# modal-labs/modal-examples

Hardware: AMD Instinct MI355X
Metric: SDXL 1024px images/sec (whole node) (higher is better)
Workload: dtype bf16; 1 GPU; model=sdxl-base-unet-2.6b, global_batch=16, image=1024x1024, denoise_steps=4, parallelism=dp1, hipgraph=True

## Files before the change

### modal_examples_amd/ops/csrc/attention_fwd32.hip

```cpp
#include "attention_mfma32.h"

#include <cstdlib>

#define FA32_NWAVES 4

template <int D, bool CAUSAL, int KVB, bool DEFER>
__global__ __launch_bounds__(FA32_NWAVES * WAVE)
__attribute__((amdgpu_waves_per_eu((D == 64 && CAUSAL) ? 3 : 1)))
void fa32_kernel(
    const short* __restrict__ Q, const short* __restrict__ K,
    const short* __restrict__ V, short* __restrict__ O,
    float* __restrict__ LSE, int B, int Hq, int Hkv, int Sq, int Sk,
    float scale, AttnFwdStrides st) {
  constexpr int KROW = D + FA_PPAD;
  constexpr int DCH = D / 16;
  constexpr int DT = D / 32;
  constexpr int QBLK = 32 * FA32_NWAVES;
  constexpr int KF = KVB / 32;

  __shared__ alignas(16) short Ks[KVB][KROW];
  __shared__ alignas(16) short Vs[KVB][KROW];

  const int tid = threadIdx.x;
  const int w = tid / WAVE;
  const int l = tid % WAVE;
  const int l31 = l & 31;
  const int hi5 = l >> 5;

  const int qblk = blockIdx.x;
  const int h = blockIdx.y;
  const int b = blockIdx.z;
  const int hkv = h / (Hq / Hkv);

  const long long qoff = b * st.q.b + h * st.q.h;
  const long long koff = b * st.k.b + hkv * st.k.h;
  const long long voff = b * st.v.b + hkv * st.v.h;
  const long long ooff = b * st.o.b + h * st.o.h;
  const int q0 = qblk * QBLK + w * 32;
  const int my_q = q0 + l31;
  const int causal_off = Sk - Sq;

  bf16x8 qreg[DCH];
  const long long qrow_off = qoff + (long long)my_q * st.q.s;
  const bool q_ok = my_q < Sq;
#pragma unroll
  for (int c = 0; c < DCH; ++c) {
    qreg[c] = q_ok
        ? *(const bf16x8*)&Q[qrow_off + c * 16 + hi5 * 8]
        : bf16x8_zero();
  }

  f32x16 acc[DT];
#pragma unroll
  for (int dt = 0; dt < DT; ++dt)
#pragma unroll
    for (int r = 0; r < 16; ++r) acc[dt][r] = 0.f;
  float m_run = -1e30f, l_run = 0.f;

  int nkb = (Sk + KVB - 1) / KVB;
  if (CAUSAL) {
    int max_kv = qblk * QBLK + QBLK - 1 + causal_off;
    int lim = (max_kv + KVB) / KVB;
    if (lim < nkb) nkb = lim;
  }

  constexpr int NT = FA32_NWAVES * WAVE;
  bf16x8 kreg[KVB * (D / 8) / NT], vreg[KVB * (D / 8) / NT];
  auto load_chunks = [&](int kb) {
    stage_load<D, KVB, NT>(K + koff, st.k.s, V + voff, st.v.s, kb * KVB, Sk,
                           tid, kreg, vreg);
  };
  auto write_chunks = [&]() {
    stage_write<D, KVB, NT>(&Ks[0][0], &Vs[0][0], tid, kreg, vreg);
  };

  load_chunks(0);
  for (int kb = 0; kb < nkb; ++kb) {
    __syncthreads();
    write_chunks();
    __syncthreads();
    if (kb + 1 < nkb) load_chunks(kb + 1);

    f32x16 s[KF];
#pragma unroll
    for (int f = 0; f < KF; ++f)
#pragma unroll
      for (int r = 0; r < 16; ++r) s[f][r] = 0.f;
#pragma unroll
    for (int f = 0; f < KF; ++f) {
#pragma unroll
      for (int c = 0; c < DCH; ++c) {
        bf16x8 kfrag = row_frag<KROW>(&Ks[0][0], f * 32 + l31, hi5, c);
        __builtin_amdgcn_s_setprio(1);
        s[f] = __builtin_amdgcn_mfma_f32_32x32x16_bf16(kfrag, qreg[c], s[f], 0,
                                                       0, 0);
        __builtin_amdgcn_s_setprio(0);
      }
    }

    bool full = (kb * KVB + KVB <= Sk) &&
                (!CAUSAL || kb * KVB + KVB - 1 <= my_q + causal_off);
#pragma unroll
    for (int f = 0; f < KF; ++f)
#pragma unroll
      for (int r = 0; r < 16; ++r) {
        int kvp = kb * KVB + f * 32 + c_row(r, hi5);
        bool dead = !full && ((kvp >= Sk) || (CAUSAL && kvp > my_q + causal_off));
        s[f][r] = dead ? -1e30f : s[f][r] * scale;
      }
    float smax = s[0][0];
#pragma unroll
    for (int f = 0; f < KF; ++f)
#pragma unroll
      for (int r = 0; r < 16; ++r) smax = fmaxf(smax, s[f][r]);
    smax = fmaxf(smax, __shfl_xor(smax, 32, WAVE));
    if (!DEFER || kb == 0 ||
        __ballot(smax > m_run + 8.f) != 0ull) {
      float m_new = fmaxf(m_run, smax);
      float rs = __expf(m_run - m_new);
      if (kb > 0 && __ballot(rs < 0.999999f) != 0ull) {
        l_run *= rs;
#pragma unroll
        for (int dt = 0; dt < DT; ++dt)
#pragma unroll
          for (int r = 0; r < 16; ++r) acc[dt][r] *= rs;
      }
      m_run = m_new;
    }
    float psum = 0.f;
#pragma unroll
    for (int f = 0; f < KF; ++f)
#pragma unroll
      for (int r = 0; r < 16; ++r) {
        s[f][r] = __expf(s[f][r] - m_run);
        psum += s[f][r];
      }
    psum += __shfl_xor(psum, 32, WAVE);
    l_run = (kb == 0) ? psum : l_run + psum;

    bf16x8 pfrag[2 * KF];
#pragma unroll
    for (int c = 0; c < 2 * KF; ++c)
      pfrag[c] = c8_to_bfrag((const float*)&s[c >> 1] + (c & 1) * 8);

#pragma unroll
    for (int c = 0; c < 2 * KF; ++c) {
#pragma unroll
      for (int dt = 0; dt < DT; ++dt) {
        bf16x8 vfrag = tr_frag<KROW>(&Vs[0][0], l, hi5, c, dt);
        __builtin_amdgcn_s_setprio(1);
        acc[dt] = __builtin_amdgcn_mfma_f32_32x32x16_bf16(vfrag, pfrag[c],
                                                          acc[dt], 0, 0, 0);
        __builtin_amdgcn_s_setprio(0);
      }
    }
  }

  if (my_q < Sq) {
    const bool hidden = CAUSAL && my_q + causal_off < 0;
    if (LSE != nullptr && hi5 == 0)
      LSE[((long long)b * Hq + h) * Sq + my_q] =
          hidden ? -INFINITY : m_run + logf(l_run);
    float inv = l_run > 0.f ? 1.f / l_run : 0.f;
#pragma unroll
    for (int dt = 0; dt < DT; ++dt)
#pragma unroll
      for (int r = 0; r < 16; ++r) {
        int d = dt * 32 + c_row(r, hi5);
        O[ooff + (long long)my_q * st.o.s + d] =
            f2bf(hidden ? 0.f : acc[dt][r] * inv);
      }
  }
}

extern "C" int fa32_fwd_strided_bf16(
    const void* q, const void* k, const void* v, void* o, float* lse, int B,
    int Hq, int Hkv, int Sq, int Sk, int D, float scale, int causal,
    const long long* strides, hipStream_t stream) {
  if (!attn_mfma32_supported(D, Hq, Hkv)) return 1;
  const short* Qp = (const short*)q;
  const short* Kp = (const short*)k;
  const short* Vp = (const short*)v;
  short* Op = (short*)o;
  const AttnFwdStrides st = attn_strides_from<AttnFwdStrides>(strides);
  dim3 grid((Sq + 127) / 128, Hq, B);
  dim3 block(FA32_NWAVES * WAVE);
  static const bool defer_env = getenv("MODAL_AMD_FA_NODEFER") == nullptr;
#define L32K(DD, CC, KK)                                                      \
  do {                                                                        \
    if (defer_env)                                                            \
      hipLaunchKernelGGL((fa32_kernel<DD, CC, KK, true>), grid, block, 0,     \
                         stream, Qp, Kp, Vp, Op, lse, B, Hq, Hkv, Sq, Sk,     \
                         scale, st);                                          \
    else                                                                      \
      hipLaunchKernelGGL((fa32_kernel<DD, CC, KK, false>), grid, block, 0,    \
                         stream, Qp, Kp, Vp, Op, lse, B, Hq, Hkv, Sq, Sk,     \
                         scale, st);                                          \
  } while (0)
  if (D == 64) {
    if (causal) L32K(64, true, 64); else L32K(64, false, 64);
  } else {
    if (causal) L32K(128, true, 32); else L32K(128, false, 32);
  }
#undef L32K
  return 0;
}
```

### modal_examples_amd/ops/csrc/attention_mfma32.h

```cpp
#pragma once

#include "common.h"

#include <cstring>

#define FA_PPAD 8

typedef __attribute__((ext_vector_type(16))) float f32x16;
typedef __attribute__((ext_vector_type(2))) int i32x2;
typedef __attribute__((address_space(3))) bf16x4* lds_tr_ptr;

DEV_INLINE bf16x8 bf16x8_zero() { return bf16x8{0, 0, 0, 0, 0, 0, 0, 0}; }

DEV_INLINE int tile_swz(int row, int byte_off) {
  return byte_off ^ (((row >> 3) & 3) << 4);
}

DEV_INLINE unsigned cvt_pk_bf16(float lo, float hi) {
  unsigned r;
  asm volatile("v_cvt_pk_bf16_f32 %0, %1, %2" : "=v"(r) : "v"(lo), "v"(hi));
  return r;
}

DEV_INLINE int c_row(int r, int hi5) {
  return (r & 3) + 8 * (r >> 2) + 4 * hi5;
}

template <int KROW>
DEV_INLINE bf16x8 row_frag(const short* tile, int row, int hi5, int c) {
  return *(const bf16x8*)((const char*)tile + row * (KROW * 2) +
                          tile_swz(row, (c * 16 + hi5 * 8) * 2));
}

template <int KROW>
DEV_INLINE bf16x8 tr_frag(const short* tile, int l, int hi5, int c, int dt) {
  int row0 = c * 16 + hi5 * 8 + ((l & 15) >> 2);
  int dbase = dt * 32 + ((l >> 4) & 1) * 16 + ((l & 3) * 4);
  bf16x4 lo = __builtin_amdgcn_ds_read_tr16_b64_v4i16((lds_tr_ptr)(
      (char*)tile + row0 * (KROW * 2) + tile_swz(row0, dbase * 2)));
  bf16x4 hi = __builtin_amdgcn_ds_read_tr16_b64_v4i16((lds_tr_ptr)(
      (char*)tile + (row0 + 4) * (KROW * 2) + tile_swz(row0 + 4, dbase * 2)));
  bf16x8 f;
#pragma unroll
  for (int j = 0; j < 4; ++j) {
    f[j] = lo[j];
    f[j + 4] = hi[j];
  }
  return f;
}

DEV_INLINE bf16x8 c8_to_bfrag(const float* sv) {
  int pk01 = (int)cvt_pk_bf16(sv[0], sv[1]);
  int pk23 = (int)cvt_pk_bf16(sv[2], sv[3]);
  int pk45 = (int)cvt_pk_bf16(sv[4], sv[5]);
  int pk67 = (int)cvt_pk_bf16(sv[6], sv[7]);
  i32x2 x = __builtin_amdgcn_permlane32_swap(pk01, pk45, false, false);
  i32x2 y = __builtin_amdgcn_permlane32_swap(pk23, pk67, false, false);
  union {
    int w[4];
    bf16x8 v;
  } u;
  u.w[0] = x[0];
  u.w[1] = y[0];
  u.w[2] = x[1];
  u.w[3] = y[1];
  return u.v;
}

template <int D, int ROWS, int NT>
DEV_INLINE void stage_load(const short* a, long long a_rs, const short* b,
                           long long b_rs, int row0, int nrows, int tid,
                           bf16x8 (&ra)[ROWS * (D / 8) / NT],
                           bf16x8 (&rb)[ROWS * (D / 8) / NT]) {
  constexpr int CPR = D / 8;
#pragma unroll
  for (int i = 0; i < ROWS * CPR / NT; ++i) {
    int ci = i * NT + tid;
    int row = ci / CPR, c8 = ci % CPR;
    int gr = row0 + row;
    if (gr < nrows) {
      ra[i] = *(const bf16x8*)&a[gr * a_rs + c8 * 8];
      rb[i] = *(const bf16x8*)&b[gr * b_rs + c8 * 8];
    } else {
      ra[i] = bf16x8_zero();
      rb[i] = bf16x8_zero();
    }
  }
}

template <int D, int ROWS, int NT>
DEV_INLINE void stage_write(short* ta, short* tb, int tid,
                            const bf16x8 (&ra)[ROWS * (D / 8) / NT],
                            const bf16x8 (&rb)[ROWS * (D / 8) / NT]) {
  constexpr int CPR = D / 8;
#pragma unroll
  for (int i = 0; i < ROWS * CPR / NT; ++i) {
    int ci = i * NT + tid;
    int row = ci / CPR, c8 = ci % CPR;
    int off = row * ((D + FA_PPAD) * 2) + tile_swz(row, c8 * 16);
    *(bf16x8*)((char*)ta + off) = ra[i];
    *(bf16x8*)((char*)tb + off) = rb[i];
  }
}

struct AttnStride {
  long long b, h, s;
};
struct AttnFwdStrides {
  AttnStride q, k, v, o;
};
struct AttnBwdStrides {
  AttnStride q, k, v, o, g, dq, dk, dv;
};

template <typename S>
inline S attn_strides_from(const long long* flat) {
  static_assert(sizeof(S) % sizeof(AttnStride) == 0, "triples only");
  S st;
  memcpy(&st, flat, sizeof(S));
  return st;
}

inline bool attn_mfma32_supported(int D, int Hq, int Hkv) {
  return (D == 64 || D == 128) && Hkv > 0 && Hq % Hkv == 0;
}
```

Measured before the change: 19.74 images/s.

## Software-pipeline LDS fragment loads with MFMAs in fa32 attention kernel

Restructures the attention inner loop so K fragments for the next 32-row block, and V fragments for the next PV chunk, are read from LDS while the current MFMAs run, with sched_barrier fences keeping that order. The masking check becomes wave-uniform (using the readfirstlane'd q0), so fully unmasked blocks take a plain scale path. The cross-half reductions use permlane32_swap instead of shfl_xor. waves_per_eu is raised for the non-causal and D=128 variants. The cost is higher register pressure from the prefetch buffers, which, combined with the occupancy hint, could cause spills.

New measurement: 20.32 images/s, median of 6. +3.0%, better.

```diff
diff --git a/modal_examples_amd/ops/csrc/attention_fwd32.hip b/modal_examples_amd/ops/csrc/attention_fwd32.hip
--- a/modal_examples_amd/ops/csrc/attention_fwd32.hip
+++ b/modal_examples_amd/ops/csrc/attention_fwd32.hip
@@ -6,7 +6,7 @@
 
 template <int D, bool CAUSAL, int KVB, bool DEFER>
 __global__ __launch_bounds__(FA32_NWAVES * WAVE)
-__attribute__((amdgpu_waves_per_eu((D == 64 && CAUSAL) ? 3 : 1)))
+__attribute__((amdgpu_waves_per_eu(D == 64 ? 3 : 2)))
 void fa32_kernel(
     const short* __restrict__ Q, const short* __restrict__ K,
     const short* __restrict__ V, short* __restrict__ O,
@@ -38,6 +38,7 @@
   const long long ooff = b * st.o.b + h * st.o.h;
   const int q0 = qblk * QBLK + w * 32;
   const int my_q = q0 + l31;
+  const int q0w = __builtin_amdgcn_readfirstlane(q0);
   const int causal_off = Sk - Sq;
 
   bf16x8 qreg[DCH];
@@ -86,34 +87,57 @@
     for (int f = 0; f < KF; ++f)
 #pragma unroll
       for (int r = 0; r < 16; ++r) s[f][r] = 0.f;
+    bf16x8 kf[KF][DCH];
+    bf16x8 vf[2][DT];
+#pragma unroll
+    for (int c = 0; c < DCH; ++c)
+      kf[0][c] = row_frag<KROW>(&Ks[0][0], l31, hi5, c);
 #pragma unroll
     for (int f = 0; f < KF; ++f) {
-#pragma unroll
-      for (int c = 0; c < DCH; ++c) {
-        bf16x8 kfrag = row_frag<KROW>(&Ks[0][0], f * 32 + l31, hi5, c);
-        __builtin_amdgcn_s_setprio(1);
-        s[f] = __builtin_amdgcn_mfma_f32_32x32x16_bf16(kfrag, qreg[c], s[f], 0,
-                                                       0, 0);
-        __builtin_amdgcn_s_setprio(0);
-      }
-    }
-
-    bool full = (kb * KVB + KVB <= Sk) &&
-                (!CAUSAL || kb * KVB + KVB - 1 <= my_q + causal_off);
+      if (f + 1 < KF) {
+#pragma unroll
+        for (int c = 0; c < DCH; ++c)
+          kf[f + 1][c] = row_frag<KROW>(&Ks[0][0], (f + 1) * 32 + l31, hi5, c);
+      } else {
+#pragma unroll
+        for (int dt = 0; dt < DT; ++dt)
+          vf[0][dt] = tr_frag<KROW>(&Vs[0][0], l, hi5, 0, dt);
+      }
+      __builtin_amdgcn_sched_barrier(0);
+      __builtin_amdgcn_s_setprio(1);
+#pragma unroll
+      for (int c = 0; c < DCH; ++c)
+        s[f] = __builtin_amdgcn_mfma_f32_32x32x16_bf16(kf[f][c], qreg[c], s[f],
+                                                       0, 0, 0);
+      __builtin_amdgcn_s_setprio(0);
+      __builtin_amdgcn_sched_barrier(0);
+    }
+
+    const bool full = (kb * KVB + KVB <= Sk) &&
+                      (!CAUSAL || kb * KVB + KVB - 1 <= q0w + causal_off);
+    if (full) {
+#pragma unroll
+      for (int f = 0; f < KF; ++f)
+#pragma unroll
+        for (int r = 0; r < 16; ++r) s[f][r] *= scale;
+    } else {
+#pragma unroll
+      for (int f = 0; f < KF; ++f)
+#pragma unroll
+        for (int r = 0; r < 16; ++r) {
+          int kvp = kb * KVB + f * 32 + c_row(r, hi5);
+          bool dead = (kvp >= Sk) || (CAUSAL && kvp > my_q + causal_off);
+          s[f][r] = dead ? -1e30f : s[f][r] * scale;
+        }
+    }
+    float smax = s[0][0];
 #pragma unroll
     for (int f = 0; f < KF; ++f)
 #pragma unroll
-      for (int r = 0; r < 16; ++r) {
-        int kvp = kb * KVB + f * 32 + c_row(r, hi5);
-        bool dead = !full && ((kvp >= Sk) || (CAUSAL && kvp > my_q + causal_off));
-        s[f][r] = dead ? -1e30f : s[f][r] * scale;
-      }
-    float smax = s[0][0];
-#pragma unroll
-    for (int f = 0; f < KF; ++f)
-#pragma unroll
       for (int r = 0; r < 16; ++r) smax = fmaxf(smax, s[f][r]);
-    smax = fmaxf(smax, __shfl_xor(smax, 32, WAVE));
+    float pa, pb;
+    lane_pair(smax, pa, pb);
+    smax = fmaxf(pa, pb);
     if (!DEFER || kb == 0 ||
         __ballot(smax > m_run + 8.f) != 0ull) {
       float m_new = fmaxf(m_run, smax);
@@ -135,7 +159,8 @@
         s[f][r] = __expf(s[f][r] - m_run);
         psum += s[f][r];
       }
-    psum += __shfl_xor(psum, 32, WAVE);
+    lane_pair(psum, pa, pb);
+    psum = pa + pb;
     l_run = (kb == 0) ? psum : l_run + psum;
 
     bf16x8 pfrag[2 * KF];
@@ -145,14 +170,19 @@
 
 #pragma unroll
     for (int c = 0; c < 2 * KF; ++c) {
-#pragma unroll
-      for (int dt = 0; dt < DT; ++dt) {
-        bf16x8 vfrag = tr_frag<KROW>(&Vs[0][0], l, hi5, c, dt);
-        __builtin_amdgcn_s_setprio(1);
-        acc[dt] = __builtin_amdgcn_mfma_f32_32x32x16_bf16(vfrag, pfrag[c],
-                                                          acc[dt], 0, 0, 0);
-        __builtin_amdgcn_s_setprio(0);
-      }
+      if (c + 1 < 2 * KF) {
+#pragma unroll
+        for (int dt = 0; dt < DT; ++dt)
+          vf[(c + 1) & 1][dt] = tr_frag<KROW>(&Vs[0][0], l, hi5, c + 1, dt);
+      }
+      __builtin_amdgcn_sched_barrier(0);
+      __builtin_amdgcn_s_setprio(1);
+#pragma unroll
+      for (int dt = 0; dt < DT; ++dt)
+        acc[dt] = __builtin_amdgcn_mfma_f32_32x32x16_bf16(
+            vf[c & 1][dt], pfrag[c], acc[dt], 0, 0, 0);
+      __builtin_amdgcn_s_setprio(0);
+      __builtin_amdgcn_sched_barrier(0);
     }
   }
 
diff --git a/modal_examples_amd/ops/csrc/attention_mfma32.h b/modal_examples_amd/ops/csrc/attention_mfma32.h
--- a/modal_examples_amd/ops/csrc/attention_mfma32.h
+++ b/modal_examples_amd/ops/csrc/attention_mfma32.h
@@ -67,6 +67,14 @@
   return u.v;
 }
 
+DEV_INLINE void lane_pair(float x, float& lo, float& hi) {
+  int xi = __builtin_bit_cast(int, x);
+  i32x2 r = __builtin_amdgcn_permlane32_swap(xi, xi, false, false);
+  int r0 = r[0], r1 = r[1];
+  lo = __builtin_bit_cast(float, r0);
+  hi = __builtin_bit_cast(float, r1);
+}
+
 template <int D, int ROWS, int NT>
 DEV_INLINE void stage_load(const short* a, long long a_rs, const short* b,
                            long long b_rs, int row0, int nrows, int tid,
```
